# EDAPINENUT/CBGBench

Measured on NVIDIA H100. Metric: ligands/sec sampled (1000-step denoise, batch 64), higher is better.
Workload: dtype f32

## Files before the change

cbgbench_b200/_lib.py:

```python
import ctypes as C
import os

from .build import LIB_PATH

_lib = None
DEFAULT_EDGE_IMPL = 6


class SamplePlan(C.Structure):
    _fields_ = [
        ('blob', C.c_void_p), ('num_layers', C.c_int32), ('num_classes', C.c_int32),
        ('emb_wt', C.c_void_p), ('h_lig_bias', C.c_void_p), ('h_static', C.c_void_p),
        ('graph_ptr', C.c_void_p), ('n_graphs', C.c_int32), ('max_graph_nodes', C.c_int32),
        ('n_nodes', C.c_int64), ('lig_node', C.c_void_p), ('n_lig', C.c_int32),
        ('gen_lig', C.c_void_p), ('gen_node', C.c_void_p), ('n_gen', C.c_int32),
        ('mode', C.c_int32), ('k', C.c_int32), ('r_max', C.c_float),
        ('workspace', C.c_void_p), ('workspace_bytes', C.c_size_t),
        ('rcache', C.c_void_p), ('rcache_bytes', C.c_size_t), ('prune', C.c_int32), ('static_lists', C.c_int32),
    ]


class StepCoef(C.Structure):
    _fields_ = [
        ('pos_c0', C.c_float), ('pos_ct', C.c_float), ('pos_logvar', C.c_float), ('pos_nonzero', C.c_float),
# ... 42 lines not shown
    'cbg_selftest_umma_f16': (_I32, [_P, _P, _P, _I32, _P]),
    'cbg_debug_x2h_trace': (_I32, [_P, _I32]),
    'cbg_debug_node_gemm_trace': (_I32, [_P]),
    'cbg_set_option': (_I32, [C.c_char_p, _I32]),
    'cbg_profile_num_families': (_I32, []),
    'cbg_profile_family_name': (C.c_char_p, [_I32]),
    'cbg_profile_enable': (_I32, [_I32]),
    'cbg_profile_collect': (_I32, [_P, _P]),
    'cbg_blob_global_floats': (_I64, []),
    'cbg_blob_layer_floats': (_I64, []),
    'cbg_blob_num_fields': (_I32, [_I32]),
    'cbg_blob_field_name': (C.c_char_p, [_I32, _I32]),
    'cbg_blob_field_offset': (_I64, [_I32, _I32]),
    'cbg_blob_field_size': (_I64, [_I32, _I32]),
    'cbg_rcache_bytes': (_I64, [_I64, _I32]),
    'cbg_workspace_bytes': (_I64, [_I64, _I64]),
    'cbg_build_neighbors_f32': (_I32, [_P, _P, _I32, _I64, _I32, _I32, _I32, _F, _P, _P, _SZ, _P]),
    'cbg_edge_gate_f32': (_I32, [_P, _P, _P, _I64, _P, _P, _SZ, _P]),
    'cbg_denoiser_forward_f32': (_I32, [_P, _I32, _I32, _P, _P, _P, _I32, _I32, _P, _P, _P, _I32, _P, _I32,
                                        _I64, _I32, _I32, _F, _I32, _P, _P, _P, _P, _SZ, _P]),
    'cbg_denoiser_forward_host_f32': (_I32, [_P, _I64, _I64, _I32, _I32, _P, _P, _P, _I32, _P, _P, _I64,
                                             _I32, _I32, _F, _P, _P, _P]),
    'cbg_node_proj_f32': (_I32, [_P, _I32, _I32, _P, _P, _I32, _I64, _P, _P]),
    'cbg_sample_begin_f32': (_I32, [C.POINTER(SamplePlan), _P, _P, _P, _P]),
    'cbg_sample_prune_counts_host': (_I32, [C.POINTER(SamplePlan), _P, _P]),
    'cbg_sample_step_f32': (_I32, [C.POINTER(SamplePlan), C.POINTER(StepCoef), _P, _P, _P, _P, _P, _P, _P, _P, _P, _P]),
    'cbg_sample_step_graph_f32': (_I32, [C.POINTER(SamplePlan), C.POINTER(StepCoef), _P, _P, _P, _P, _P, _P, _P, _P]),
    'cbg_sample_step_graph_nodes': (_I64, [C.POINTER(SamplePlan), _P]),
    'cbg_eval_loss_f32': (_I32, [C.POINTER(SamplePlan), C.POINTER(EvalCoef), _I32, _P, _P, _P, _P, _P, _P, _P, _P, _P, _P, _P]),
    'cbg_sbdd_step_f32': (_I32, [C.POINTER(SamplePlan), C.POINTER(SbddCoef), _P, _P, _P, _P, _P, _P, _P, _P, _P]),
    'cbg_bp_step_f32': (_I32, [C.POINTER(SamplePlan), _P, _I32, C.POINTER(BpCoef), _P, _P, _P, _P, _P, _P, _P, _P, _P, _P]),
    'cbg_bp_eval_loss_f32': (_I32, [C.POINTER(SamplePlan), _P, _I32, C.POINTER(BpEvalCoef), _I32, _P, _P, _P, _P, _P, _P,
                                     _P, _P, _P, _P, _P]),
    'cbg_sbdd_eval_loss_f32': (_I32, [C.POINTER(SamplePlan), C.POINTER(SbddEvalCoef), _I32, _P, _P, _P, _P, _P, _P, _P, _P,
                                       _P, _P, _P, _P]),
    'cbg_pocket_stats_f32': (_I32, [_P, _P, _I32, _P, _P, _I32, _P, _P, _P]),
    'cbg_sample_ligand_sizes': (_I32, [_P, _P, _I32, _I32, _P, _P, _P, _P, _P, _P]),
    'cbg_build_batch_f32': (_I32, [_P, _P]),
    'cbg_ipa_head_floats': (_I64, [_I32]),
    'cbg_ipa_layer_floats': (_I64, [_I32]),
    'cbg_ipa_head_fields': (_I32, []),
    'cbg_ipa_layer_fields': (_I32, []),
    'cbg_ipa_head_field_name': (C.c_char_p, [_I32]),
    'cbg_ipa_layer_field_name': (C.c_char_p, [_I32]),
    'cbg_ipa_head_field_offset': (_I64, [_I32, _I32]),
    'cbg_ipa_head_field_size': (_I64, [_I32, _I32]),
# ... 62 lines not shown
```

cbgbench_b200/csrc/api.cu:

```cuda
#include <stdarg.h>
#include <stdio.h>
#include <stdlib.h>
#include <string.h>
#include <mutex>
#include <vector>

#include <nvtx3/nvToolsExt.h>

#include "../../include/cbg_b200.h"
#include "cbg_kernels.cuh"

long long g_cbg_launches = 0;
int g_cbg_prof_on = 0;

namespace {
struct NvtxRange {
  explicit NvtxRange(const char* name) { nvtxRangePushA(name); }
  ~NvtxRange() { nvtxRangePop(); }
};
struct ProfMark { int family; int is_end; cudaEvent_t ev; };
std::vector<ProfMark> g_prof_marks;
const char* const kFamilyNames[CBG_K_COUNT] = {"knn", "edge_gate", "node_gemm", "x2h_k", "x2h_v", "h2x",
                                               "classifier", "step_init", "reverse", "misc"};
}
// ... 122 lines not shown
                            float* const planes[CBG_NPLANES]) {
  auto field = [&](int x2h, int h2x) { return L + cbg_layout::layer_offset(sub == kX2H ? x2h : h2x); };
  const int first = shape == Planes::kDst ? 2 : 0;
  NodeGemmArgs g{};
  g.a = a; g.row_idx = row_idx; g.n_rows = n_rows;
  g.wt = field(CBG_LF_X2H_NODE_WT, CBG_LF_H2X_NODE_WT) + first * CBG_H;
  g.bias = field(CBG_LF_X2H_NODE_B, CBG_LF_H2X_NODE_B) + first * CBG_H;
  g.ldw = 640;
  g.n_planes = shape == Planes::kAll ? 5 : (shape == Planes::kSrc ? 2 : 3);
  g.has_q = shape != Planes::kSrc;
  for (int p = 0; p < g.n_planes - g.has_q; ++p) g.out[p] = planes[first + p];
  if (g.has_q) {
    g.q_ln = field(CBG_LF_X2H_Q_LN, CBG_LF_H2X_Q_LN);
    g.q_w1t = field(CBG_LF_X2H_Q_W1T, CBG_LF_H2X_Q_W1T);
    g.q_b1 = field(CBG_LF_X2H_Q_B1, CBG_LF_H2X_Q_B1);
    g.out_q = planes[4];
  }
  g.tc_planes = field(CBG_LF_X2H_NODE_TC, CBG_LF_H2X_NODE_TC); g.tc_first_plane = first;
  g.tch_planes = field(CBG_LF_X2H_NODE_TCH, CBG_LF_H2X_NODE_TCH);
  return g;
}

struct AuxStream {
  cudaStream_t s2 = nullptr, s3 = nullptr, s4 = nullptr;
  cudaEvent_t ev_h = nullptr, ev_x = nullptr, ev_h0 = nullptr, ev_p = nullptr, ev_gi = nullptr;
  int state = -1;
};
constexpr int kMaxDevices = 64;
AuxStream g_aux_dev[kMaxDevices];

AuxStream* aux_streams() {
  int dev = -1;
  if (cudaGetDevice(&dev) != cudaSuccess || dev < 0 || dev >= kMaxDevices) return nullptr;
  AuxStream& a = g_aux_dev[dev];
  if (a.state < 0) {
    a.state = switches().overlap &&
              cudaStreamCreateWithFlags(&a.s2, cudaStreamNonBlocking) == cudaSuccess &&
              cudaStreamCreateWithFlags(&a.s3, cudaStreamNonBlocking) == cudaSuccess &&
              cudaStreamCreateWithFlags(&a.s4, cudaStreamNonBlocking) == cudaSuccess &&
              cudaEventCreateWithFlags(&a.ev_h, cudaEventDisableTiming) == cudaSuccess &&
              cudaEventCreateWithFlags(&a.ev_x, cudaEventDisableTiming) == cudaSuccess &&
              cudaEventCreateWithFlags(&a.ev_h0, cudaEventDisableTiming) == cudaSuccess &&
              cudaEventCreateWithFlags(&a.ev_p, cudaEventDisableTiming) == cudaSuccess &&
              cudaEventCreateWithFlags(&a.ev_gi, cudaEventDisableTiming) == cudaSuccess;
  }
  return a.state ? &a : nullptr;
}

bool plan_prunes(const cbg_sample_plan& p) {
  return p.prune != 0 && switches().prune && p.num_layers > 0 && (p.n_gen > 0 || p.n_lig > 0);
}

int run_h2x(const float* L, const Workspace& ws, long long n_nodes, const int* gen_idx, int n_gen,
            const int* src_rows_dev, const AuxStream* aux, cudaStream_t st) {
  NodeGemmArgs gj = node_gemm_args(L, kH2X, Planes::kSrc, ws.h, src_rows_dev ? ws.order : nullptr, (int)n_nodes, ws.hplane);
  gj.n_rows_dev = src_rows_dev;
  if (int rc = launch_node_gemm(gj, st)) return rc;
  const NodeGemmArgs gi = node_gemm_args(L, kH2X, Planes::kDst, ws.h, gen_idx, n_gen, ws.hplane);
  if (int rc = launch_node_gemm(gi, aux ? aux->s4 : st)) return rc;
  if (aux) {
    CBG_CUDA_OK(cudaEventRecord(aux->ev_gi, aux->s4));
    CBG_CUDA_OK(cudaStreamWaitEvent(st, aux->ev_gi, 0));
  }
  EdgeArgs x{};
  x.x4 = ws.x4; x.nbr = ws.nbr; x.ew = ws.ew;
  x.pj_k = ws.hplane[0]; x.pj_v = ws.hplane[1]; x.pi_k = ws.hplane[2]; x.pi_v = ws.hplane[3]; x.q = ws.hplane[4];
  x.layer = L; x.h = ws.h; x.node_idx = gen_idx; x.n_nodes = n_gen; x.dx = ws.dx;
  x.w = ws.hw;
  if (int rc = cbg_launch_h2x(x, st)) return rc;
  return cbg_launch_apply_dx(ws.x4, gen_idx, ws.dx, n_gen, st);
}

int run_denoiser(const cbg_sample_plan& p, const Workspace& ws, cudaStream_t st) {
  static std::mutex core_mutex;
  std::lock_guard<std::mutex> core_lock(core_mutex);
  NvtxRange nvtx_core("cbg:denoiser");
  const long long n_nodes = p.n_nodes;
  const int num_layers = p.num_layers, n_gen = p.n_gen;
  const bool static_lists = p.static_lists != 0 || p.rcache != nullptr;
  if (n_nodes > 0x7fffffffLL / (CBG_KMAX * CBG_HEADS)) { cbg_set_error("n_nodes too large for 32-bit indexing"); return 1; }
  if (int rc = cbg_launch_knn(ws.x4, p.graph_ptr, p.n_graphs, p.max_graph_nodes, p.mode, p.k, p.r_max, 0,
                              static_lists ? ws.snbr : nullptr, ws.nbr, st)) return rc;
  const float* layers = p.blob + cbg_layout::kGlobalFloats;
  const bool prune = plan_prunes(p);
  AuxStream* const aux = n_gen > 0 ? aux_streams() : nullptr;
// ... 37 lines not shown
      NodeGemmArgs gd = node_gemm_args(L, kX2H, Planes::kDst, ws.h, ws.order, (int)n_nodes, ws.plane);
      gd.n_rows_dev = ws.cnt + l + 1;
      if (int rc = launch_node_gemm(gd, st)) return rc;
      if (aux) CBG_CUDA_OK(cudaStreamWaitEvent(st, aux->ev_p, 0));
    }
    if (aux && x_pending) { CBG_CUDA_OK(cudaStreamWaitEvent(st, aux->ev_x, 0)); x_pending = false; }
    EdgeArgs e{};
    e.x4 = ws.x4; e.nbr = ws.nbr; e.ew = ws.ew;
    e.pj_k = ws.plane[0]; e.pj_v = ws.plane[1]; e.pi_k = ws.plane[2]; e.pi_v = ws.plane[3]; e.q = ws.plane[4];
    e.layer = L; e.w = ws.w; e.h = ws.h; e.node_idx = nullptr; e.n_nodes = (int)n_nodes; e.dx = nullptr;
    if (prune) { e.node_idx = ws.order; e.n_nodes_dev = ws.cnt + l + 1; }
    if (tickets) e.ticket = ws.tickets + 2 * l;
    if (p.rcache) {
      const size_t per = (size_t)n_nodes * (CBG_KMAX * CBG_H);
      e.rc_k = p.rcache + (size_t)(2 * l) * per;
      e.rc_v = p.rcache + (size_t)(2 * l + 1) * per;
      e.fstat = switches().static_fast ? ws.fstat : nullptr;
    }
    if (int rc = cbg_launch_x2h(e, st)) return rc;
    if (n_gen <= 0) continue;
    if (aux) {
      CBG_CUDA_OK(cudaEventRecord(aux->ev_h, st));
      CBG_CUDA_OK(cudaStreamWaitEvent(sx, aux->ev_h, 0));
      CBG_CUDA_OK(cudaStreamWaitEvent(aux->s4, aux->ev_h, 0));
    }
    if (int rc = run_h2x(L, ws, n_nodes, p.gen_node, n_gen, prune ? ws.cnt + num_layers : nullptr, aux, sx)) return rc;
    if (aux) { CBG_CUDA_OK(cudaEventRecord(aux->ev_x, sx)); x_pending = true; }
  }
  if (aux && x_pending) CBG_CUDA_OK(cudaStreamWaitEvent(st, aux->ev_x, 0));
  return 0;
}

int run_bp_denoiser(const cbg_sample_plan& p, const float* com_blob, int com_layers, const Workspace& ws,
                    const float* x_t, float* logits, float* x_pred, cudaStream_t st) {
  if (int rc = run_denoiser(p, ws, st)) return rc;
  if (int rc = cbg_launch_classifier(p.blob, ws.h, p.lig_node, p.n_lig, p.num_classes, logits, st)) return rc;
  if (int rc = cbg_launch_gather_x(ws.x4, p.lig_node, p.n_lig, x_pred, st)) return rc;
  if (int rc = cbg_launch_scatter_x(x_t, p.lig_node, p.n_lig, ws.x4, st)) return rc;
  if (p.n_gen <= 0 || com_layers <= 0) return 0;
  if (int rc = cbg_launch_edge_gate_rows(com_blob, ws.x4, ws.nbr, p.gen_node, p.n_gen, ws.ew, st)) return rc;
  const int* src_rows_dev = plan_prunes(p) ? ws.cnt + p.num_layers : nullptr;
  const float* layers = com_blob + cbg_layout::kGlobalFloats;
  for (int l = 0; l < com_layers; ++l) {
    if (int rc = run_h2x(layers + (size_t)l * cbg_layout::kLayerFloats, ws, p.n_nodes, p.gen_node, p.n_gen, src_rows_dev,
                         nullptr, st)) return rc;
  }
  return 0;
}

struct BpScratch { float* logits; float* x_pred; };
BpScratch bp_scratch(const Workspace& ws, int n_lig, int num_classes) {
  return {ws.w, ws.w + align256((size_t)n_lig * num_classes * 4) / 4};
}

int open_plan(const cbg_sample_plan* plan, bool args_ok, const char* null_msg, Workspace* ws) {
  if (!plan || !args_ok) { cbg_set_error("%s", null_msg); return 1; }
  if (int rc = check_ws(plan->workspace, plan->workspace_bytes, plan->n_nodes, plan->n_gen, ws)) return rc;
  const int K = plan->num_classes;
  if (K < 1 || K > CBG_MAXCLS) { cbg_set_error("num_classes=%d outside [1,%d]", K, CBG_MAXCLS); return 1; }
  return 0;
}

int check_replicas(const cbg_sample_plan& p, int n_t, int copies = 1) {
  const int max_t = CBG_EVAL_MAX_REPLICAS / copies;
  if (n_t < 1 || n_t > max_t) { cbg_set_error("%s=%d outside [1,%d]", copies == 1 ? "n_rep" : "n_t", n_t, max_t); return 1; }
  const int n_rep = n_t * copies;
  if (p.n_lig < n_rep || p.n_lig % n_rep || p.n_graphs % n_rep) {
    cbg_set_error("plan (n_lig=%d, n_graphs=%d) is not %d replicas of one batch", p.n_lig, p.n_graphs, n_rep); return 1;
// ... 215 lines not shown
                                        (const float*)(d + o_h), (const int32_t*)(d + o_gp), n_graphs,
                                        max_graph_nodes, (const uint8_t*)(d + o_lf), (const uint8_t*)(d + o_gf),
                                        (const int32_t*)(d + o_gi), n_gen, nullptr, 0, n_nodes, mode, k, r_max, -1,
                                        (float*)(d + o_xo), (float*)(d + o_ho), (float*)(d + o_lo), d, ws_bytes, st))
    return rc;
  if (x_out_host) CBG_CUDA_OK(cudaMemcpyAsync(x_out_host, d + o_xo, (size_t)n_nodes * 12, cudaMemcpyDeviceToHost, st));
  if (h_out_host) CBG_CUDA_OK(cudaMemcpyAsync(h_out_host, d + o_ho, (size_t)n_nodes * CBG_H * 4, cudaMemcpyDeviceToHost, st));
  if (logits_out_host) CBG_CUDA_OK(cudaMemcpyAsync(logits_out_host, d + o_lo, (size_t)n_nodes * num_classes * 4, cudaMemcpyDeviceToHost, st));
  CBG_CUDA_OK(cudaStreamSynchronize(st));
  return 0;
}

int32_t cbg_node_proj_f32(const float* blob_layer, int32_t sublayer, int32_t impl, const float* h,
                          const int32_t* row_idx, int32_t n_rows, int64_t n_nodes, float* planes, void* stream) {
  if (sublayer < 0 || sublayer > 1 || (impl != 0 && impl != 1 && impl != 2 && impl != 11 && impl != 12 && impl != 14)) { cbg_set_error("bad sublayer/impl"); return 1; }
  float* out[CBG_NPLANES];
  for (int p = 0; p < CBG_NPLANES; ++p) out[p] = planes + (size_t)p * n_nodes * CBG_H;
  const NodeGemmArgs g = node_gemm_args(blob_layer, (SubLayer)sublayer, Planes::kAll, h, row_idx, n_rows, out);
  if (impl == 0) return cbg_launch_node_gemm(g, (cudaStream_t)stream);
  if (impl == 2) return cbg_launch_node_gemm_f16(g, (cudaStream_t)stream);
  return cbg_launch_node_gemm_tc(g, (cudaStream_t)stream, impl == 12 ? 2 : (impl == 14 ? 4 : (impl == 11 ? 1 : 0)));
}

int32_t cbg_sample_begin_f32(const cbg_sample_plan* plan, const float* x_nodes, const uint8_t* lig_flag,
                             const uint8_t* gen_flag, void* stream) {
  if (!plan) { cbg_set_error("null plan"); return 1; }
  Workspace ws;
  if (int rc = check_ws(plan->workspace, plan->workspace_bytes, plan->n_nodes, plan->n_gen, &ws)) return rc;
  cudaStream_t st = (cudaStream_t)stream;
  if (int rc = cbg_launch_pack_x4(x_nodes, lig_flag, gen_flag, plan->n_nodes, ws.x4, st)) return rc;
  if (plan->rcache || plan->static_lists) {
    if (int rc = cbg_launch_knn(ws.x4, plan->graph_ptr, plan->n_graphs, plan->max_graph_nodes, CBG_MODE_KNN, CBG_KMAX,
                                0.f, 1, nullptr, ws.snbr, st)) return rc;
    if (int rc = cbg_launch_edge_gate(plan->blob, ws.x4, ws.snbr, plan->n_nodes, nullptr, nullptr, ws.sew, st)) return rc;
  }
  if (plan->rcache) {
    const int64_t need = cbg_rcache_bytes(plan->n_nodes, plan->num_layers);
    if ((int64_t)plan->rcache_bytes < need) { cbg_set_error("rcache too small: have %zu bytes, need %lld", plan->rcache_bytes, (long long)need); return 1; }
    if (int rc = cbg_launch_rcache(plan->blob + cbg_layout::kGlobalFloats, plan->num_layers, ws.x4, ws.snbr,
                                   (int)plan->n_nodes, plan->rcache, st)) return rc;
  }
  return 0;
}

int32_t cbg_sample_prune_counts_host(const cbg_sample_plan* plan, int32_t* counts_host, void* stream) {
  if (!plan || !counts_host) { cbg_set_error("cbg_sample_prune_counts_host: null argument"); return 1; }
// ... 350 lines not shown
```

cbgbench_b200/csrc/cbg_kernels.cuh:

```cuda
#pragma once
#include "cbg_common.cuh"

#define CBG_MODE_KNN 0
#define CBG_MODE_RADIUS 1

int cbg_launch_knn(const float4* x4, const int* graph_ptr, int n_graphs, int max_graph_nodes, int mode,
                   int k, float r_max, int static_only, const int* snbr, int* nbr, cudaStream_t st);
int cbg_launch_edge_gate(const float* blob_global, const float4* x4, const int* nbr, long long n_nodes,
                         const float* ew_static, int* glist, float* ew, cudaStream_t st,
                         unsigned char* full_static = nullptr);

int cbg_launch_depth(const int* nbr, const int* graph_ptr, int n_graphs, int max_graph_nodes, long long n_nodes,
                     const int* seed_idx, int n_seed, const int* cls_idx, int n_cls, int num_layers,
                     int* depth, int* order, int* cnt_ge, cudaStream_t st);

struct NodeGemmArgs {
  const float* a;
  const int* row_idx;
  int n_rows;
  const float* wt;
  const float* bias;
  int ldw;
  int n_planes;
  float* out[CBG_NPLANES];
  int has_q;
  const float* q_ln;
  const float* q_w1t;
  const float* q_b1;
  float* out_q;
  const int* n_rows_dev;
  const float* tc_planes;
  int tc_first_plane;
  const float* tch_planes;
  const int* n_dst_dev;
  long long* trace;
};
int cbg_launch_node_gemm(const NodeGemmArgs& a, cudaStream_t st);
int cbg_launch_node_gemm_tc(const NodeGemmArgs& a, cudaStream_t st, int cluster = 0);
int cbg_launch_node_gemm_f16(const NodeGemmArgs& a, cudaStream_t st);
void cbg_node_gemm_f16_set_trace(long long* buf_dev);

struct EdgeArgs {
  const float4* x4;
  const int* nbr;
  const float* ew;
  const float* pj_k;
  const float* pj_v;
  const float* pi_k;
  const float* pi_v;
  const float* q;
  const float* layer;
  float* w;
  float* h;
  const int* node_idx;
  int n_nodes;
  float* dx;
  const int* n_nodes_dev;
  const float* rc_k;
  const float* rc_v;
  int* ticket;
  const unsigned char* fstat;
  long long* trace;
// ... 212 lines not shown
```

cbgbench_b200/csrc/node_gemm_f16.cu:

```cuda
#include "cbg_kernels.cuh"
#include "cbg_tc.cuh"

using namespace cbg_tc;

namespace {

constexpr int TM = 128;
constexpr int KC = 64;
constexpr int NKC = CBG_H / KC;
constexpr int STAGES = 3;
constexpr uint32_t A_TILE = TM * CBG_H * 2;
constexpr uint32_t B_CHUNK = 128 * KC * 2;
constexpr uint32_t B_STAGE = 2 * B_CHUNK;
constexpr uint32_t SM_A_HI = 0;
constexpr uint32_t SM_Q = 2 * A_TILE;
constexpr uint32_t SM_B0 = 4 * A_TILE;
constexpr uint32_t SM_BARS = SM_B0 + STAGES * B_STAGE;
constexpr uint32_t SM_TOTAL = SM_BARS + 64;
static_assert(SM_TOTAL <= 232448, "shared memory budget");
constexpr uint32_t A_SBO = (CBG_H / 8) * 128, B_SBO = (KC / 8) * 128, LBO = 128;
constexpr float kScaleA = 16.f;
constexpr float kInvAcc = 1.f / 4096.f;

__device__ __forceinline__ uint32_t a_off8(int row, int k8) {
  return (uint32_t)(row >> 3) * A_SBO + (uint32_t)k8 * 128u + (uint32_t)(row & 7) * 16u;
}
__device__ __forceinline__ void store_split8(uint8_t* tile, int row, int k8, const float4 a, const float4 b) {
  uint4 hi, lo;
  split_pair(a.x * kScaleA, a.y * kScaleA, hi.x, lo.x);
  split_pair(a.z * kScaleA, a.w * kScaleA, hi.y, lo.y);
  split_pair(b.x * kScaleA, b.y * kScaleA, hi.z, lo.z);
  split_pair(b.z * kScaleA, b.w * kScaleA, hi.w, lo.w);
  const uint32_t off = a_off8(row, k8);
  *reinterpret_cast<uint4*>(tile + off) = hi;
  *reinterpret_cast<uint4*>(tile + A_TILE + off) = lo;
}

struct Sched {
  int n_gemm, n_norm, has_q;
  __device__ __forceinline__ Sched(const NodeGemmArgs& p, bool cta_dst) {
    has_q = (p.has_q && cta_dst) ? 1 : 0;
    if (cta_dst) n_norm = p.n_planes - (p.has_q ? 1 : 0);
    else { n_norm = CBG_NODE_SRC_PLANES - p.tc_first_plane; n_norm = n_norm < 0 ? 0 : (n_norm > p.n_planes ? p.n_planes : n_norm); }
    n_gemm = n_norm + 2 * has_q;
  }
  __device__ __forceinline__ int kind(int g) const { return has_q ? (g == 0 ? 1 : (g == n_gemm - 1 ? 2 : 0)) : 0; }
  __device__ __forceinline__ int rel(const NodeGemmArgs& p, int g) const {
    if (has_q && g == 0) return p.n_planes - 1;
    if (has_q && g == n_gemm - 1) return -1;
    const int idx = has_q ? g - 1 : g;
    return n_norm > 1 ? (idx + (int)(blockIdx.x % (unsigned)n_norm)) % n_norm : idx;
  }
};
__device__ __forceinline__ const float* chunk_src(const NodeGemmArgs& p, const Sched& sc, int i) {
  const int g = i / NKC, c = i % NKC;
  const int r = sc.rel(p, g);
  const int plane = r < 0 ? 5 : p.tc_first_plane + r;
  return p.tch_planes + (size_t)plane * (NKC * B_STAGE / 4) + (size_t)c * (B_STAGE / 4);
}

__device__ __forceinline__ void stamp(long long* trace, int slot) {
  if (trace && blockIdx.x == 0) {
    unsigned long long t;
    asm volatile("mov.u64 %0, %%globaltimer;" : "=l"(t));
    trace[slot] = (long long)t;
  }
}

__device__ __forceinline__ float quad_sum(float v) {
  v += __shfl_xor_sync(CBG_FULL, v, 1);
  return v + __shfl_xor_sync(CBG_FULL, v, 2);
}

__global__ void __launch_bounds__(288, 1) node_gemm_f16_kernel(const __grid_constant__ NodeGemmArgs p) {
  extern __shared__ __align__(1024) uint8_t smem[];
  const int tid = threadIdx.x, warp = tid >> 5, lane = tid & 31;
  int n_rows = p.n_rows;
  if (p.n_rows_dev) { const int nd = *p.n_rows_dev; n_rows = nd < n_rows ? nd : n_rows; }
  int n_dst = n_rows;
  if (p.n_dst_dev) { const int nd = *p.n_dst_dev; n_dst = nd < n_dst ? nd : n_dst; }
  const int row0 = blockIdx.x * TM;
  if (row0 >= n_rows) return;
  const Sched sc(p, row0 < n_dst);
  if (sc.n_gemm == 0) return;
  const uint32_t sbase = smem_u32(smem);
  const uint32_t bar_full = sbase + SM_BARS;
  const uint32_t bar_empty = bar_full + 8 * STAGES;
  const int total_chunks = sc.n_gemm * NKC;
  if (tid == 0) stamp(p.trace, 0);

  if (tid == 256) {
    for (int s = 0; s < STAGES; ++s) { mbar_init(bar_full + 8 * s, 1); mbar_init(bar_empty + 8 * s, 2); }
    fence_mbar_init();
    for (int i = 0; i < STAGES && i < total_chunks; ++i) {
      mbar_expect_tx(bar_full + 8 * i, B_STAGE);
      bulk_g2s(sbase + SM_B0 + i * B_STAGE, chunk_src(p, sc, i), B_STAGE, bar_full + 8 * i);
    }
  }
  if (warp < 8) {
    const int r = tid & (TM - 1);
    const int row = row0 + r;
    const bool live = row < n_rows;
    const float* arow = p.a + (size_t)(live ? (p.row_idx ? p.row_idx[row] : row) : 0) * CBG_H;
    const float4 z = make_float4(0.f, 0.f, 0.f, 0.f);
    float4 v[16];
#pragma unroll
    for (int j = 0; j < 8; ++j) {
      const int k8 = (tid >> 7) + 2 * j;
      v[2 * j] = live ? ldg4(arow + 8 * k8) : z;
      v[2 * j + 1] = live ? ldg4(arow + 8 * k8 + 4) : z;
    }
#pragma unroll
    for (int j = 0; j < 8; ++j) store_split8(smem + SM_A_HI, r, (tid >> 7) + 2 * j, v[2 * j], v[2 * j + 1]);
    fence_proxy_async();
  }
  __syncthreads();
  if (tid == 0) stamp(p.trace, 1);

  if (warp == 8) {
    if (lane == 0) {
      for (int i = STAGES; i < total_chunks; ++i) {
        const int s = i % STAGES;
        mbar_wait(bar_empty + 8 * s, (uint32_t)(((i / STAGES) - 1) & 1));
        mbar_expect_tx(bar_full + 8 * s, B_STAGE);
        bulk_g2s(sbase + SM_B0 + s * B_STAGE, chunk_src(p, sc, i), B_STAGE, bar_full + 8 * s);
      }
    }
    return;
  }
  const int wg = warp >> 2, qg = lane >> 2, qt = lane & 3;
  const int r_lo = 64 * wg + 16 * (warp & 3) + qg;
  int node[2];
#pragma unroll
  for (int h = 0; h < 2; ++h) {
    const int grow = row0 + r_lo + 8 * h;
    node[h] = (grow < n_rows) ? (p.row_idx ? p.row_idx[grow] : grow) : -1;
  }
  for (int g = 0; g < sc.n_gemm; ++g) {
    const int kind = sc.kind(g), rel = sc.rel(p, g);
    const uint32_t a_base = sbase + (kind == 2 ? SM_Q : SM_A_HI) + (uint32_t)(8 * wg) * A_SBO;
    const uint64_t da_hi = smem_desc(a_base, LBO, A_SBO), da_lo = smem_desc(a_base + A_TILE, LBO, A_SBO);
    float d[64];
#pragma unroll
    for (int c = 0; c < NKC; ++c) {
      const int i = g * NKC + c, s = i % STAGES;
      mbar_wait(bar_full + 8 * s, (uint32_t)((i / STAGES) & 1));
      const uint64_t db_hi = smem_desc(sbase + SM_B0 + s * B_STAGE, LBO, B_SBO);
      const uint64_t db_lo = smem_desc(sbase + SM_B0 + s * B_STAGE + B_CHUNK, LBO, B_SBO);
      wgmma_fence();
#pragma unroll
      for (int ks = 0; ks < KC / 16; ++ks) {
        const uint64_t ka = (uint64_t)(16 * (c * (KC / 16) + ks)), kb = (uint64_t)(16 * ks);
        wgmma_f16_ss(d, da_lo + ka, db_hi + kb, (c == 0 && ks == 0) ? 0u : 1u);
        wgmma_f16_ss(d, da_hi + ka, db_lo + kb, 1u);
        wgmma_f16_ss(d, da_hi + ka, db_hi + kb, 1u);
      }
      wgmma_commit();
      wgmma_wait0();
      if ((tid & 127) == 0) mbar_arrive(bar_empty + 8 * s);
    }
    wgmma_settle(d);
    if (tid == 0) stamp(p.trace, 2 + g);
    if (kind != 1) {
      const float* bias = kind == 2 ? p.q_b1 : p.bias + rel * CBG_H;
      float* out = kind == 2 ? p.out_q : p.out[rel];
      const bool dst_plane = kind == 2 || p.tc_first_plane + rel >= CBG_NODE_SRC_PLANES;
      const int row_lim = dst_plane ? n_dst : n_rows;
#pragma unroll
      for (int h = 0; h < 2; ++h) {
        if (node[h] < 0 || row0 + r_lo + 8 * h >= row_lim) continue;
        float* o = out + (size_t)node[h] * CBG_H + 2 * qt;
#pragma unroll
        for (int j = 0; j < 16; ++j) {
          const float2 b = __ldg(reinterpret_cast<const float2*>(bias + 8 * j + 2 * qt));
          *reinterpret_cast<float2*>(o + 8 * j) = make_float2(fmaf(d[4 * j + 2 * h], kInvAcc, b.x), fmaf(d[4 * j + 2 * h + 1], kInvAcc, b.y));
        }
      }
    } else {
      const float* bias = p.bias + rel * CBG_H;
      float s0 = 0.f, s1 = 0.f;
#pragma unroll
      for (int j = 0; j < 16; ++j) {
        const float2 b = __ldg(reinterpret_cast<const float2*>(bias + 8 * j + 2 * qt));
        d[4 * j] = fmaf(d[4 * j], kInvAcc, b.x);
        d[4 * j + 1] = fmaf(d[4 * j + 1], kInvAcc, b.y);
        d[4 * j + 2] = fmaf(d[4 * j + 2], kInvAcc, b.x);
        d[4 * j + 3] = fmaf(d[4 * j + 3], kInvAcc, b.y);
        s0 += d[4 * j] + d[4 * j + 1];
        s1 += d[4 * j + 2] + d[4 * j + 3];
      }
      const float mean0 = quad_sum(s0) * (1.f / 128.f), mean1 = quad_sum(s1) * (1.f / 128.f);
      float q0 = 0.f, q1 = 0.f;
#pragma unroll
      for (int j = 0; j < 16; ++j) {
        d[4 * j] -= mean0; d[4 * j + 1] -= mean0; d[4 * j + 2] -= mean1; d[4 * j + 3] -= mean1;
        q0 = fmaf(d[4 * j], d[4 * j], q0); q0 = fmaf(d[4 * j + 1], d[4 * j + 1], q0);
        q1 = fmaf(d[4 * j + 2], d[4 * j + 2], q1); q1 = fmaf(d[4 * j + 3], d[4 * j + 3], q1);
      }
      const float rstd0 = 1.f / sqrtf(quad_sum(q0) * (1.f / 128.f) + 1e-5f);
      const float rstd1 = 1.f / sqrtf(quad_sum(q1) * (1.f / 128.f) + 1e-5f);
#pragma unroll
      for (int j = 0; j < 16; ++j) {
        const float2 gm = __ldg(reinterpret_cast<const float2*>(p.q_ln + 8 * j + 2 * qt));
        const float2 bt = __ldg(reinterpret_cast<const float2*>(p.q_ln + 128 + 8 * j + 2 * qt));
#pragma unroll
        for (int h = 0; h < 2; ++h) {
          const float rs = h ? rstd1 : rstd0;
          const float a0 = fmaxf(fmaf(d[4 * j + 2 * h] * rs, gm.x, bt.x), 0.f);
          const float a1 = fmaxf(fmaf(d[4 * j + 2 * h + 1] * rs, gm.y, bt.y), 0.f);
          uint32_t hi, lo;
          split_pair(a0 * kScaleA, a1 * kScaleA, hi, lo);
          const uint32_t off = a_off8(r_lo + 8 * h, j) + 4u * (uint32_t)qt;
          *reinterpret_cast<uint32_t*>(smem + SM_Q + off) = hi;
          *reinterpret_cast<uint32_t*>(smem + SM_Q + A_TILE + off) = lo;
        }
      }
      fence_proxy_async();
      warpgroup_sync(wg);
    }
    if (tid == 0) stamp(p.trace, 10 + g);
  }
  if (tid == 0) stamp(p.trace, 20);
}

}

static long long* g_trace_buf = nullptr;
void cbg_node_gemm_f16_set_trace(long long* buf_dev) { g_trace_buf = buf_dev; }

int cbg_launch_node_gemm_f16(const NodeGemmArgs& a, cudaStream_t st) {
  if (a.n_rows <= 0) return 0;
  if (!a.tch_planes) { cbg_set_error("f16 tensor-core node GEMM needs the f16 weight images (tch_planes)"); return 1; }
  static bool attr_dev[CBG_MAX_DEVICES] = {};
  bool& attr_set = cbg_dev_flag(attr_dev);
  if (!attr_set) {
    CBG_CUDA_OK(cudaFuncSetAttribute(node_gemm_f16_kernel, cudaFuncAttributeMaxDynamicSharedMemorySize, (int)SM_TOTAL));
    attr_set = true;
  }
  NodeGemmArgs args = a;
  args.trace = g_trace_buf;
  CBG_PROF_BEGIN(CBG_K_NODE_GEMM, st);
  node_gemm_f16_kernel<<<(a.n_rows + TM - 1) / TM, 288, SM_TOTAL, st>>>(args);
  CBG_LAUNCHED(CBG_K_NODE_GEMM, st);
  return 0;
}
```

include/cbg_b200.h:

```cpp
#ifndef CBG_B200_H_
#define CBG_B200_H_

#include <stddef.h>
#include <stdint.h>

#ifdef __cplusplus
extern "C" {
#endif

#define CBG_NBR_WIDTH 32
#define CBG_HIDDEN 128
#define CBG_N_HEADS 16
#define CBG_MAX_CLASSES 16

#define CBG_CUTOFF_KNN 0
#define CBG_CUTOFF_RADIUS 1

int32_t cbg_version(void);
const char* cbg_last_error(void);
int64_t cbg_launch_count(void);

int32_t cbg_profile_num_families(void);
const char* cbg_profile_family_name(int32_t i);
int32_t cbg_profile_enable(int32_t on);
// ... 27 lines not shown
                          void* workspace, size_t workspace_bytes, void* stream);

int32_t cbg_denoiser_forward_f32(const float* blob, int32_t num_layers, int32_t num_classes,
                                 const float* x , const float* h ,
                                 const int32_t* graph_ptr, int32_t n_graphs, int32_t max_graph_nodes,
                                 const uint8_t* lig_flag , const uint8_t* gen_flag ,
                                 const int32_t* gen_idx, int32_t n_gen,
                                 const int32_t* cls_idx, int32_t n_cls,
                                 int64_t n_nodes, int32_t mode, int32_t k, float r_max,
                                 int32_t stop_after_layers,
                                 float* x_out , float* h_out , float* logits_out,
                                 void* workspace, size_t workspace_bytes, void* stream);

int32_t cbg_denoiser_forward_host_f32(const float* blob_host, int64_t blob_floats, int64_t blob_version,
                                      int32_t num_layers, int32_t num_classes,
                                      const float* x_host, const float* h_host,
                                      const int32_t* graph_ptr_host, int32_t n_graphs,
                                      const uint8_t* lig_flag_host, const uint8_t* gen_flag_host,
                                      int64_t n_nodes, int32_t mode, int32_t k, float r_max,
                                      float* x_out_host, float* h_out_host, float* logits_out_host);

int32_t cbg_node_proj_f32(const float* blob_layer, int32_t sublayer, int32_t impl, const float* h,
                          const int32_t* row_idx, int32_t n_rows, int64_t n_nodes, float* planes, void* stream);

typedef struct cbg_sample_plan {
  const float* blob;
  int32_t num_layers;
  int32_t num_classes;
  const float* emb_wt;
  const float* h_lig_bias;
  const float* h_static;
  const int32_t* graph_ptr;
  int32_t n_graphs;
  int32_t max_graph_nodes;
  int64_t n_nodes;
  const int32_t* lig_node;
  int32_t n_lig;
  const uint8_t* gen_lig;
  const int32_t* gen_node;
  int32_t n_gen;
  int32_t mode;
  int32_t k;
  float r_max;
  void* workspace;
  size_t workspace_bytes;
  float* rcache;
// ... 192 lines not shown
```

Measured before the change: 13.99.

## Make f16 node GEMM persistent and fuse src/dst H2X jobs into one launch

The f16 tensor-core node GEMM becomes a persistent kernel with grid equal to the SM count. Each CTA takes a contiguous, weight-balanced range of (job, tile, plane) GEMMs drawn from up to two jobs and restages the A tile whenever the tile changes. H2X now submits its src and dst projections as one fused launch when node_gemm==2, replacing the separate aux stream s4 and its events. This cuts launch count and cross-stream syncs and balances work across SMs, but drops the separate Q A-tile buffer, so A is restaged more often and the scheduling logic gets more complex.

After: 14.25, median of 6. 1.02x the previous value.

```diff
diff --git a/cbgbench_b200/_lib.py b/cbgbench_b200/_lib.py
--- a/cbgbench_b200/_lib.py
+++ b/cbgbench_b200/_lib.py
@@ -88,6 +88,7 @@
     'cbg_denoiser_forward_host_f32': (_I32, [_P, _I64, _I64, _I32, _I32, _P, _P, _P, _I32, _P, _P, _I64,
                                              _I32, _I32, _F, _P, _P, _P]),
     'cbg_node_proj_f32': (_I32, [_P, _I32, _I32, _P, _P, _I32, _I64, _P, _P]),
+    'cbg_debug_node_gemm_jobs': (_I32, [_P, _I32, _P, _I64, _P, _I32, _P, _P, _P, _P, _P, _P]),
     'cbg_sample_begin_f32': (_I32, [C.POINTER(SamplePlan), _P, _P, _P, _P]),
     'cbg_sample_prune_counts_host': (_I32, [C.POINTER(SamplePlan), _P, _P]),
     'cbg_sample_step_f32': (_I32, [C.POINTER(SamplePlan), C.POINTER(StepCoef), _P, _P, _P, _P, _P, _P, _P, _P, _P, _P]),
diff --git a/cbgbench_b200/csrc/api.cu b/cbgbench_b200/csrc/api.cu
--- a/cbgbench_b200/csrc/api.cu
+++ b/cbgbench_b200/csrc/api.cu
@@ -168,8 +168,8 @@
 }
 
 struct AuxStream {
-  cudaStream_t s2 = nullptr, s3 = nullptr, s4 = nullptr;
-  cudaEvent_t ev_h = nullptr, ev_x = nullptr, ev_h0 = nullptr, ev_p = nullptr, ev_gi = nullptr;
+  cudaStream_t s2 = nullptr, s3 = nullptr;
+  cudaEvent_t ev_h = nullptr, ev_x = nullptr, ev_h0 = nullptr, ev_p = nullptr;
   int state = -1;
 };
 constexpr int kMaxDevices = 64;
@@ -183,12 +183,10 @@
     a.state = switches().overlap &&
               cudaStreamCreateWithFlags(&a.s2, cudaStreamNonBlocking) == cudaSuccess &&
               cudaStreamCreateWithFlags(&a.s3, cudaStreamNonBlocking) == cudaSuccess &&
-              cudaStreamCreateWithFlags(&a.s4, cudaStreamNonBlocking) == cudaSuccess &&
               cudaEventCreateWithFlags(&a.ev_h, cudaEventDisableTiming) == cudaSuccess &&
               cudaEventCreateWithFlags(&a.ev_x, cudaEventDisableTiming) == cudaSuccess &&
               cudaEventCreateWithFlags(&a.ev_h0, cudaEventDisableTiming) == cudaSuccess &&
-              cudaEventCreateWithFlags(&a.ev_p, cudaEventDisableTiming) == cudaSuccess &&
-              cudaEventCreateWithFlags(&a.ev_gi, cudaEventDisableTiming) == cudaSuccess;
+              cudaEventCreateWithFlags(&a.ev_p, cudaEventDisableTiming) == cudaSuccess;
   }
   return a.state ? &a : nullptr;
 }
@@ -198,15 +196,15 @@
 }
 
 int run_h2x(const float* L, const Workspace& ws, long long n_nodes, const int* gen_idx, int n_gen,
-            const int* src_rows_dev, const AuxStream* aux, cudaStream_t st) {
+            const int* src_rows_dev, cudaStream_t st) {
   NodeGemmArgs gj = node_gemm_args(L, kH2X, Planes::kSrc, ws.h, src_rows_dev ? ws.order : nullptr, (int)n_nodes, ws.hplane);
   gj.n_rows_dev = src_rows_dev;
-  if (int rc = launch_node_gemm(gj, st)) return rc;
   const NodeGemmArgs gi = node_gemm_args(L, kH2X, Planes::kDst, ws.h, gen_idx, n_gen, ws.hplane);
-  if (int rc = launch_node_gemm(gi, aux ? aux->s4 : st)) return rc;
-  if (aux) {
-    CBG_CUDA_OK(cudaEventRecord(aux->ev_gi, aux->s4));
-    CBG_CUDA_OK(cudaStreamWaitEvent(st, aux->ev_gi, 0));
+  if (switches().node_gemm == 2) {
+    if (int rc = cbg_launch_node_gemm_f16(gj, st, &gi)) return rc;
+  } else {
+    if (int rc = launch_node_gemm(gj, st)) return rc;
+    if (int rc = launch_node_gemm(gi, st)) return rc;
   }
   EdgeArgs x{};
   x.x4 = ws.x4; x.nbr = ws.nbr; x.ew = ws.ew;
@@ -290,9 +288,8 @@
     if (aux) {
       CBG_CUDA_OK(cudaEventRecord(aux->ev_h, st));
       CBG_CUDA_OK(cudaStreamWaitEvent(sx, aux->ev_h, 0));
-      CBG_CUDA_OK(cudaStreamWaitEvent(aux->s4, aux->ev_h, 0));
     }
-    if (int rc = run_h2x(L, ws, n_nodes, p.gen_node, n_gen, prune ? ws.cnt + num_layers : nullptr, aux, sx)) return rc;
+    if (int rc = run_h2x(L, ws, n_nodes, p.gen_node, n_gen, prune ? ws.cnt + num_layers : nullptr, sx)) return rc;
     if (aux) { CBG_CUDA_OK(cudaEventRecord(aux->ev_x, sx)); x_pending = true; }
   }
   if (aux && x_pending) CBG_CUDA_OK(cudaStreamWaitEvent(st, aux->ev_x, 0));
@@ -311,7 +308,7 @@
   const float* layers = com_blob + cbg_layout::kGlobalFloats;
   for (int l = 0; l < com_layers; ++l) {
     if (int rc = run_h2x(layers + (size_t)l * cbg_layout::kLayerFloats, ws, p.n_nodes, p.gen_node, p.n_gen, src_rows_dev,
-                         nullptr, st)) return rc;
+                         st)) return rc;
   }
   return 0;
 }
@@ -573,6 +570,24 @@
   return cbg_launch_node_gemm_tc(g, (cudaStream_t)stream, impl == 12 ? 2 : (impl == 14 ? 4 : (impl == 11 ? 1 : 0)));
 }
 
+int32_t cbg_debug_node_gemm_jobs(const float* blob_layer, int32_t sublayer, const float* h, int64_t n_nodes, float* planes,
+                                 int32_t n_jobs, const int32_t* shape, const int32_t* const* row_idx, const int32_t* n_rows,
+                                 const int32_t* const* n_rows_dev, const int32_t* const* n_dst_dev, void* stream) {
+  if (sublayer < 0 || sublayer > 1 || n_jobs < 1 || n_jobs > 2 || !shape || !n_rows) {
+    cbg_set_error("cbg_debug_node_gemm_jobs: bad sublayer / n_jobs / arguments"); return 1;
+  }
+  float* out[CBG_NPLANES];
+  for (int p = 0; p < CBG_NPLANES; ++p) out[p] = planes + (size_t)p * n_nodes * CBG_H;
+  NodeGemmArgs g[2];
+  for (int j = 0; j < n_jobs; ++j) {
+    if (shape[j] < 0 || shape[j] > 2) { cbg_set_error("cbg_debug_node_gemm_jobs: shape %d", shape[j]); return 1; }
+    g[j] = node_gemm_args(blob_layer, (SubLayer)sublayer, (Planes)shape[j], h, row_idx ? row_idx[j] : nullptr, n_rows[j], out);
+    g[j].n_rows_dev = n_rows_dev ? n_rows_dev[j] : nullptr;
+    g[j].n_dst_dev = n_dst_dev ? n_dst_dev[j] : nullptr;
+  }
+  return cbg_launch_node_gemm_f16(g[0], (cudaStream_t)stream, n_jobs > 1 ? &g[1] : nullptr);
+}
+
 int32_t cbg_sample_begin_f32(const cbg_sample_plan* plan, const float* x_nodes, const uint8_t* lig_flag,
                              const uint8_t* gen_flag, void* stream) {
   if (!plan) { cbg_set_error("null plan"); return 1; }
diff --git a/cbgbench_b200/csrc/cbg_kernels.cuh b/cbgbench_b200/csrc/cbg_kernels.cuh
--- a/cbgbench_b200/csrc/cbg_kernels.cuh
+++ b/cbgbench_b200/csrc/cbg_kernels.cuh
@@ -33,11 +33,10 @@
   int tc_first_plane;
   const float* tch_planes;
   const int* n_dst_dev;
-  long long* trace;
 };
 int cbg_launch_node_gemm(const NodeGemmArgs& a, cudaStream_t st);
 int cbg_launch_node_gemm_tc(const NodeGemmArgs& a, cudaStream_t st, int cluster = 0);
-int cbg_launch_node_gemm_f16(const NodeGemmArgs& a, cudaStream_t st);
+int cbg_launch_node_gemm_f16(const NodeGemmArgs& a, cudaStream_t st, const NodeGemmArgs* b = nullptr);
 void cbg_node_gemm_f16_set_trace(long long* buf_dev);
 
 struct EdgeArgs {
diff --git a/cbgbench_b200/csrc/node_gemm_f16.cu b/cbgbench_b200/csrc/node_gemm_f16.cu
--- a/cbgbench_b200/csrc/node_gemm_f16.cu
+++ b/cbgbench_b200/csrc/node_gemm_f16.cu
@@ -9,18 +9,25 @@
 constexpr int KC = 64;
 constexpr int NKC = CBG_H / KC;
 constexpr int STAGES = 3;
+constexpr int MAX_JOBS = 2;
 constexpr uint32_t A_TILE = TM * CBG_H * 2;
 constexpr uint32_t B_CHUNK = 128 * KC * 2;
 constexpr uint32_t B_STAGE = 2 * B_CHUNK;
-constexpr uint32_t SM_A_HI = 0;
-constexpr uint32_t SM_Q = 2 * A_TILE;
-constexpr uint32_t SM_B0 = 4 * A_TILE;
+constexpr uint32_t SM_A = 0;
+constexpr uint32_t SM_B0 = 2 * A_TILE;
 constexpr uint32_t SM_BARS = SM_B0 + STAGES * B_STAGE;
 constexpr uint32_t SM_TOTAL = SM_BARS + 64;
 static_assert(SM_TOTAL <= 232448, "shared memory budget");
 constexpr uint32_t A_SBO = (CBG_H / 8) * 128, B_SBO = (KC / 8) * 128, LBO = 128;
 constexpr float kScaleA = 16.f;
 constexpr float kInvAcc = 1.f / 4096.f;
+constexpr int kTraceGemms = 30;
+
+struct NodeGemmJobs {
+  NodeGemmArgs job[MAX_JOBS];
+  int n_jobs;
+  long long* trace;
+};
 
 __device__ __forceinline__ uint32_t a_off8(int row, int k8) {
   return (uint32_t)(row >> 3) * A_SBO + (uint32_t)k8 * 128u + (uint32_t)(row & 7) * 16u;
@@ -36,35 +43,91 @@
   *reinterpret_cast<uint4*>(tile + A_TILE + off) = lo;
 }
 
-struct Sched {
-  int n_gemm, n_norm, has_q;
-  __device__ __forceinline__ Sched(const NodeGemmArgs& p, bool cta_dst) {
-    has_q = (p.has_q && cta_dst) ? 1 : 0;
-    if (cta_dst) n_norm = p.n_planes - (p.has_q ? 1 : 0);
-    else { n_norm = CBG_NODE_SRC_PLANES - p.tc_first_plane; n_norm = n_norm < 0 ? 0 : (n_norm > p.n_planes ? p.n_planes : n_norm); }
-    n_gemm = n_norm + 2 * has_q;
-  }
-  __device__ __forceinline__ int kind(int g) const { return has_q ? (g == 0 ? 1 : (g == n_gemm - 1 ? 2 : 0)) : 0; }
-  __device__ __forceinline__ int rel(const NodeGemmArgs& p, int g) const {
-    if (has_q && g == 0) return p.n_planes - 1;
-    if (has_q && g == n_gemm - 1) return -1;
-    const int idx = has_q ? g - 1 : g;
-    return n_norm > 1 ? (idx + (int)(blockIdx.x % (unsigned)n_norm)) % n_norm : idx;
-  }
+struct JobShape {
+  int n_rows, n_dst;
+  int n_tiles, n_dtiles;
+  int n_norm_dst, has_q;
+  int n_norm_src;
+  int weight;
 };
-__device__ __forceinline__ const float* chunk_src(const NodeGemmArgs& p, const Sched& sc, int i) {
-  const int g = i / NKC, c = i % NKC;
-  const int r = sc.rel(p, g);
-  const int plane = r < 0 ? 5 : p.tc_first_plane + r;
+__device__ __forceinline__ JobShape job_shape(const NodeGemmArgs& p) {
+  JobShape s;
+  int n = p.n_rows;
+  if (p.n_rows_dev) { const int nd = *p.n_rows_dev; n = nd < n ? nd : n; }
+  n = n > 0 ? n : 0;
+  int nd = n;
+  if (p.n_dst_dev) { const int v = *p.n_dst_dev; nd = v < nd ? v : nd; }
+  nd = nd > 0 ? nd : 0;
+  s.n_rows = n; s.n_dst = nd;
+  s.n_tiles = (n + TM - 1) / TM; s.n_dtiles = (nd + TM - 1) / TM;
+  s.has_q = p.has_q ? 1 : 0;
+  s.n_norm_dst = p.n_planes - s.has_q;
+  const int ns = CBG_NODE_SRC_PLANES - p.tc_first_plane;
+  s.n_norm_src = ns < 0 ? 0 : (ns > p.n_planes ? p.n_planes : ns);
+  s.weight = s.n_dtiles * (s.n_norm_dst + 2 * s.has_q) + (s.n_tiles - s.n_dtiles) * s.n_norm_src;
+  return s;
+}
+
+struct Gemm {
+  int job, tile, kind, rel;
+  bool valid;
+};
+
+struct GemmSeq {
+  const NodeGemmJobs& P;
+  const JobShape* sh;
+  int job, tile, u, pos, end;
+  bool more;
+  bool q_second;
+
+  __device__ __forceinline__ int n_norm(int j, int t) const { return t < sh[j].n_dtiles ? sh[j].n_norm_dst : sh[j].n_norm_src; }
+  __device__ __forceinline__ int has_q(int j, int t) const { return t < sh[j].n_dtiles ? sh[j].has_q : 0; }
+  __device__ __forceinline__ void skip_empty() {
+    while (job < P.n_jobs && (tile >= sh[job].n_tiles || n_norm(job, tile) + has_q(job, tile) == 0)) { ++job; tile = 0; u = 0; }
+  }
+  __device__ __forceinline__ GemmSeq(const NodeGemmJobs& P_, const JobShape* sh_, int lo, int hi)
+      : P(P_), sh(sh_), job(0), tile(0), u(0), pos(lo), end(hi), more(false), q_second(false) {
+    int base = 0;
+    while (job < P.n_jobs && lo >= base + sh[job].weight) { base += sh[job].weight; ++job; }
+    if (job >= P.n_jobs || lo >= hi) return;
+    const JobShape& s = sh[job];
+    const int p = lo - base, wd = s.n_norm_dst + 2 * s.has_q;
+    int off;
+    if (p < s.n_dtiles * wd) { tile = p / wd; off = p - tile * wd; }
+    else { const int p2 = p - s.n_dtiles * wd; tile = s.n_dtiles + p2 / s.n_norm_src; off = p2 - (tile - s.n_dtiles) * s.n_norm_src; }
+    if (off <= n_norm(job, tile)) u = off;
+    else { ++tile; u = 0; ++pos; skip_empty(); }
+    more = job < P.n_jobs && pos < end;
+  }
+  __device__ __forceinline__ Gemm next() {
+    Gemm g;
+    g.valid = true;
+    if (q_second) {
+      q_second = false;
+      g.job = job_q; g.tile = tile_q; g.kind = 2; g.rel = -1;
+      return g;
+    }
+    if (!more) { g.valid = false; return g; }
+    const int nn = n_norm(job, tile);
+    g.job = job; g.tile = tile;
+    g.kind = u == nn ? 1 : 0;
+    g.rel = g.kind ? P.job[job].n_planes - 1 : u;
+    if (g.kind) { q_second = true; job_q = job; tile_q = tile; }
+    pos += g.kind ? 2 : 1;
+    if (++u == nn + has_q(job, tile)) { u = 0; ++tile; skip_empty(); }
+    more = job < P.n_jobs && pos < end;
+    return g;
+  }
+  int job_q = 0, tile_q = 0;
+};
+
+__device__ __forceinline__ const float* chunk_src(const NodeGemmArgs& p, const Gemm& g, int c) {
+  const int plane = g.kind == 2 ? 5 : p.tc_first_plane + g.rel;
   return p.tch_planes + (size_t)plane * (NKC * B_STAGE / 4) + (size_t)c * (B_STAGE / 4);
 }
 
 __device__ __forceinline__ void stamp(long long* trace, int slot) {
-  if (trace && blockIdx.x == 0) {
-    unsigned long long t;
-    asm volatile("mov.u64 %0, %%globaltimer;" : "=l"(t));
-    trace[slot] = (long long)t;
-  }
+  if (trace && blockIdx.x == 0) trace[slot] = (long long)global_timer_ns();
 }
 
 __device__ __forceinline__ float quad_sum(float v) {
@@ -72,78 +135,76 @@
   return v + __shfl_xor_sync(CBG_FULL, v, 2);
 }
 
-__global__ void __launch_bounds__(288, 1) node_gemm_f16_kernel(const __grid_constant__ NodeGemmArgs p) {
+__device__ __forceinline__ void stage_a(uint8_t* tile, const NodeGemmArgs& p, int n_rows, int row0, int wg, int t) {
+  const int r = 64 * wg + (t & 63), k0 = t >> 6;
+  const int row = row0 + r;
+  const bool live = row < n_rows;
+  const float* arow = p.a + (size_t)(live ? (p.row_idx ? p.row_idx[row] : row) : 0) * CBG_H;
+  const float4 z = make_float4(0.f, 0.f, 0.f, 0.f);
+  float4 v[16];
+#pragma unroll
+  for (int j = 0; j < 8; ++j) {
+    const int k8 = k0 + 2 * j;
+    v[2 * j] = live ? ldg4(arow + 8 * k8) : z;
+    v[2 * j + 1] = live ? ldg4(arow + 8 * k8 + 4) : z;
+  }
+#pragma unroll
+  for (int j = 0; j < 8; ++j) store_split8(tile, r, k0 + 2 * j, v[2 * j], v[2 * j + 1]);
+}
+
+__global__ void __launch_bounds__(288, 1) node_gemm_f16_kernel(const __grid_constant__ NodeGemmJobs P) {
   extern __shared__ __align__(1024) uint8_t smem[];
+  __shared__ JobShape sh[MAX_JOBS];
   const int tid = threadIdx.x, warp = tid >> 5, lane = tid & 31;
-  int n_rows = p.n_rows;
-  if (p.n_rows_dev) { const int nd = *p.n_rows_dev; n_rows = nd < n_rows ? nd : n_rows; }
-  int n_dst = n_rows;
-  if (p.n_dst_dev) { const int nd = *p.n_dst_dev; n_dst = nd < n_dst ? nd : n_dst; }
-  const int row0 = blockIdx.x * TM;
-  if (row0 >= n_rows) return;
-  const Sched sc(p, row0 < n_dst);
-  if (sc.n_gemm == 0) return;
+  if (tid == 0) stamp(P.trace, 0);
+  if (tid < MAX_JOBS) sh[tid] = tid < P.n_jobs ? job_shape(P.job[tid]) : JobShape{};
   const uint32_t sbase = smem_u32(smem);
   const uint32_t bar_full = sbase + SM_BARS;
   const uint32_t bar_empty = bar_full + 8 * STAGES;
-  const int total_chunks = sc.n_gemm * NKC;
-  if (tid == 0) stamp(p.trace, 0);
-
   if (tid == 256) {
     for (int s = 0; s < STAGES; ++s) { mbar_init(bar_full + 8 * s, 1); mbar_init(bar_empty + 8 * s, 2); }
     fence_mbar_init();
-    for (int i = 0; i < STAGES && i < total_chunks; ++i) {
-      mbar_expect_tx(bar_full + 8 * i, B_STAGE);
-      bulk_g2s(sbase + SM_B0 + i * B_STAGE, chunk_src(p, sc, i), B_STAGE, bar_full + 8 * i);
-    }
-  }
-  if (warp < 8) {
-    const int r = tid & (TM - 1);
-    const int row = row0 + r;
-    const bool live = row < n_rows;
-    const float* arow = p.a + (size_t)(live ? (p.row_idx ? p.row_idx[row] : row) : 0) * CBG_H;
-    const float4 z = make_float4(0.f, 0.f, 0.f, 0.f);
-    float4 v[16];
-#pragma unroll
-    for (int j = 0; j < 8; ++j) {
-      const int k8 = (tid >> 7) + 2 * j;
-      v[2 * j] = live ? ldg4(arow + 8 * k8) : z;
-      v[2 * j + 1] = live ? ldg4(arow + 8 * k8 + 4) : z;
-    }
-#pragma unroll
-    for (int j = 0; j < 8; ++j) store_split8(smem + SM_A_HI, r, (tid >> 7) + 2 * j, v[2 * j], v[2 * j + 1]);
-    fence_proxy_async();
   }
   __syncthreads();
-  if (tid == 0) stamp(p.trace, 1);
+  const int total = sh[0].weight + sh[1].weight;
+  const int lo = (int)((long long)blockIdx.x * total / gridDim.x);
+  const int hi = (int)((long long)(blockIdx.x + 1) * total / gridDim.x);
+  GemmSeq seq(P, sh, lo, hi);
 
   if (warp == 8) {
     if (lane == 0) {
-      for (int i = STAGES; i < total_chunks; ++i) {
-        const int s = i % STAGES;
-        mbar_wait(bar_empty + 8 * s, (uint32_t)(((i / STAGES) - 1) & 1));
-        mbar_expect_tx(bar_full + 8 * s, B_STAGE);
-        bulk_g2s(sbase + SM_B0 + s * B_STAGE, chunk_src(p, sc, i), B_STAGE, bar_full + 8 * s);
+      int i = 0;
+      for (Gemm g = seq.next(); g.valid; g = seq.next()) {
+        for (int c = 0; c < NKC; ++c, ++i) {
+          const int s = i % STAGES;
+          if (i >= STAGES) mbar_wait(bar_empty + 8 * s, (uint32_t)(((i / STAGES) - 1) & 1));
+          mbar_expect_tx(bar_full + 8 * s, B_STAGE);
+          bulk_g2s(sbase + SM_B0 + s * B_STAGE, chunk_src(P.job[g.job], g, c), B_STAGE, bar_full + 8 * s);
+        }
       }
     }
     return;
   }
   const int wg = warp >> 2, qg = lane >> 2, qt = lane & 3;
   const int r_lo = 64 * wg + 16 * (warp & 3) + qg;
-  int node[2];
-#pragma unroll
-  for (int h = 0; h < 2; ++h) {
-    const int grow = row0 + r_lo + 8 * h;
-    node[h] = (grow < n_rows) ? (p.row_idx ? p.row_idx[grow] : grow) : -1;
-  }
-  for (int g = 0; g < sc.n_gemm; ++g) {
-    const int kind = sc.kind(g), rel = sc.rel(p, g);
-    const uint32_t a_base = sbase + (kind == 2 ? SM_Q : SM_A_HI) + (uint32_t)(8 * wg) * A_SBO;
-    const uint64_t da_hi = smem_desc(a_base, LBO, A_SBO), da_lo = smem_desc(a_base + A_TILE, LBO, A_SBO);
+  const uint32_t a_base = sbase + SM_A + (uint32_t)(8 * wg) * A_SBO;
+  const uint64_t da_hi = smem_desc(a_base, LBO, A_SBO), da_lo = smem_desc(a_base + A_TILE, LBO, A_SBO);
+  int i = 0, n_done = 0, cur_job = -1, cur_tile = -1;
+  for (Gemm g = seq.next(); g.valid; g = seq.next(), ++n_done) {
+    const NodeGemmArgs& p = P.job[g.job];
+    const JobShape& js = sh[g.job];
+    const int row0 = g.tile * TM;
+    if (g.job != cur_job || g.tile != cur_tile) {
+      stage_a(smem + SM_A, p, js.n_rows, row0, wg, tid & 127);
+      fence_proxy_async();
+      warpgroup_sync(wg);
+      cur_job = g.job; cur_tile = g.tile;
+      if (tid == 0 && n_done == 0) stamp(P.trace, 1);
+    }
     float d[64];
 #pragma unroll
-    for (int c = 0; c < NKC; ++c) {
-      const int i = g * NKC + c, s = i % STAGES;
+    for (int c = 0; c < NKC; ++c, ++i) {
+      const int s = i % STAGES;
       mbar_wait(bar_full + 8 * s, (uint32_t)((i / STAGES) & 1));
       const uint64_t db_hi = smem_desc(sbase + SM_B0 + s * B_STAGE, LBO, B_SBO);
       const uint64_t db_lo = smem_desc(sbase + SM_B0 + s * B_STAGE + B_CHUNK, LBO, B_SBO);
@@ -160,16 +221,17 @@
       if ((tid & 127) == 0) mbar_arrive(bar_empty + 8 * s);
     }
     wgmma_settle(d);
-    if (tid == 0) stamp(p.trace, 2 + g);
-    if (kind != 1) {
-      const float* bias = kind == 2 ? p.q_b1 : p.bias + rel * CBG_H;
-      float* out = kind == 2 ? p.out_q : p.out[rel];
-      const bool dst_plane = kind == 2 || p.tc_first_plane + rel >= CBG_NODE_SRC_PLANES;
-      const int row_lim = dst_plane ? n_dst : n_rows;
+    if (tid == 0 && n_done < kTraceGemms) stamp(P.trace, 4 + 2 * n_done);
+    if (g.kind != 1) {
+      const float* bias = g.kind == 2 ? p.q_b1 : p.bias + g.rel * CBG_H;
+      float* out = g.kind == 2 ? p.out_q : p.out[g.rel];
+      const bool dst_plane = g.kind == 2 || p.tc_first_plane + g.rel >= CBG_NODE_SRC_PLANES;
+      const int row_lim = dst_plane ? js.n_dst : js.n_rows;
 #pragma unroll
       for (int h = 0; h < 2; ++h) {
-        if (node[h] < 0 || row0 + r_lo + 8 * h >= row_lim) continue;
-        float* o = out + (size_t)node[h] * CBG_H + 2 * qt;
+        const int grow = row0 + r_lo + 8 * h;
+        if (grow >= row_lim) continue;
+        float* o = out + (size_t)(p.row_idx ? p.row_idx[grow] : grow) * CBG_H + 2 * qt;
 #pragma unroll
         for (int j = 0; j < 16; ++j) {
           const float2 b = __ldg(reinterpret_cast<const float2*>(bias + 8 * j + 2 * qt));
@@ -177,7 +239,7 @@
         }
       }
     } else {
-      const float* bias = p.bias + rel * CBG_H;
+      const float* bias = p.bias + g.rel * CBG_H;
       float s0 = 0.f, s1 = 0.f;
 #pragma unroll
       for (int j = 0; j < 16; ++j) {
@@ -211,16 +273,16 @@
           uint32_t hi, lo;
           split_pair(a0 * kScaleA, a1 * kScaleA, hi, lo);
           const uint32_t off = a_off8(r_lo + 8 * h, j) + 4u * (uint32_t)qt;
-          *reinterpret_cast<uint32_t*>(smem + SM_Q + off) = hi;
-          *reinterpret_cast<uint32_t*>(smem + SM_Q + A_TILE + off) = lo;
+          *reinterpret_cast<uint32_t*>(smem + SM_A + off) = hi;
+          *reinterpret_cast<uint32_t*>(smem + SM_A + A_TILE + off) = lo;
         }
       }
       fence_proxy_async();
       warpgroup_sync(wg);
     }
-    if (tid == 0) stamp(p.trace, 10 + g);
-  }
-  if (tid == 0) stamp(p.trace, 20);
+    if (tid == 0 && n_done < kTraceGemms) stamp(P.trace, 5 + 2 * n_done);
+  }
+  if (tid == 0 && P.trace && blockIdx.x == 0) { stamp(P.trace, 2); P.trace[3] = n_done; }
 }
 
 }
@@ -228,19 +290,30 @@
 static long long* g_trace_buf = nullptr;
 void cbg_node_gemm_f16_set_trace(long long* buf_dev) { g_trace_buf = buf_dev; }
 
-int cbg_launch_node_gemm_f16(const NodeGemmArgs& a, cudaStream_t st) {
-  if (a.n_rows <= 0) return 0;
-  if (!a.tch_planes) { cbg_set_error("f16 tensor-core node GEMM needs the f16 weight images (tch_planes)"); return 1; }
-  static bool attr_dev[CBG_MAX_DEVICES] = {};
-  bool& attr_set = cbg_dev_flag(attr_dev);
-  if (!attr_set) {
+int cbg_launch_node_gemm_f16(const NodeGemmArgs& a, cudaStream_t st, const NodeGemmArgs* b) {
+  NodeGemmJobs jobs{};
+  long long max_weight = 0;
+  for (const NodeGemmArgs* j : {&a, b}) {
+    if (!j || j->n_rows <= 0) continue;
+    if (!j->tch_planes) { cbg_set_error("f16 tensor-core node GEMM needs the f16 weight images (tch_planes)"); return 1; }
+    max_weight += (long long)((j->n_rows + TM - 1) / TM) * (j->n_planes + (j->has_q ? 1 : 0));
+    jobs.job[jobs.n_jobs++] = *j;
+  }
+  if (jobs.n_jobs == 0 || max_weight == 0) return 0;
+  if (max_weight > 0x7fffffffLL) { cbg_set_error("node GEMM: too many rows"); return 1; }
+  static int sms_dev[CBG_MAX_DEVICES] = {};
+  int dev = 0;
+  CBG_CUDA_OK(cudaGetDevice(&dev));
+  if (dev < 0 || dev >= CBG_MAX_DEVICES) { cbg_set_error("device %d out of range", dev); return 1; }
+  int& sms = sms_dev[dev];
+  if (sms == 0) {
     CBG_CUDA_OK(cudaFuncSetAttribute(node_gemm_f16_kernel, cudaFuncAttributeMaxDynamicSharedMemorySize, (int)SM_TOTAL));
-    attr_set = true;
-  }
-  NodeGemmArgs args = a;
-  args.trace = g_trace_buf;
+    CBG_CUDA_OK(cudaDeviceGetAttribute(&sms, cudaDevAttrMultiProcessorCount, dev));
+  }
+  jobs.trace = g_trace_buf;
+  const int grid = (int)(max_weight < sms ? max_weight : sms);
   CBG_PROF_BEGIN(CBG_K_NODE_GEMM, st);
-  node_gemm_f16_kernel<<<(a.n_rows + TM - 1) / TM, 288, SM_TOTAL, st>>>(args);
+  node_gemm_f16_kernel<<<grid, 288, SM_TOTAL, st>>>(jobs);
   CBG_LAUNCHED(CBG_K_NODE_GEMM, st);
   return 0;
 }
diff --git a/include/cbg_b200.h b/include/cbg_b200.h
--- a/include/cbg_b200.h
+++ b/include/cbg_b200.h
@@ -73,6 +73,9 @@
 
 int32_t cbg_node_proj_f32(const float* blob_layer, int32_t sublayer, int32_t impl, const float* h,
                           const int32_t* row_idx, int32_t n_rows, int64_t n_nodes, float* planes, void* stream);
+int32_t cbg_debug_node_gemm_jobs(const float* blob_layer, int32_t sublayer, const float* h, int64_t n_nodes, float* planes,
+                                 int32_t n_jobs, const int32_t* shape, const int32_t* const* row_idx, const int32_t* n_rows,
+                                 const int32_t* const* n_rows_dev, const int32_t* const* n_dst_dev, void* stream);
 
 typedef struct cbg_sample_plan {
   const float* blob;
```
